# yurimjeon1892/EFGH

Measured on AMD Instinct MI355X. Metric: frame-pairs/sec EFGHNet fwd+bwd (384x1280 RGB + 64x2048 range), whole job, higher is better.
Workload: dtype f32; 1 GPU; BASELINE.json configs[2]: EFGHNet fwd+bwd with efghloss + gradient all-reduce + fused Adam, synthetic 384x1280 RGB + 131072-point sweep, batch=8 per GPU, random-init weights; global_batch=8, points=131072, parallelism=dp1

## Files before the change

### efgh_amd/csrc/gemm.hip

```cpp
#include "common.h"
#include <type_traits>

namespace {

typedef float f32x16 __attribute__((ext_vector_type(16)));
constexpr int BK = 32;
constexpr int LDS_LD = BK + 4;
struct KArgs {
    const float *A; int64_t lda;
    int C, T, K;
    unsigned magicC;
    int Hin, Win, Hv, Wv, sh, sw;
    unsigned long long dhpack, dwpack;
    int Ho, Wo, osh, osw, oh0, ow0;
    const int *table;
    const float *W; int N;
    int tld;
    long long M; const int *M_dev;
    const float *bias, *scale, *shift, *residual; int64_t ldr;
    int act; float slope;
    float *out; int64_t ldo;
    float *stats;
    unsigned nbx;
    unsigned nbatch;
// ... 73 lines not shown
    if (p.stats) {
#pragma unroll
        for (int j = 0; j < NI; ++j) {
            const int coll = (wn * NI + j) * 32 + l31;
            s1[j] += __shfl_xor(s1[j], 32); s2[j] += __shfl_xor(s2[j], 32);
            if (lh == 0) { ssum[wm * BN + coll] = s1[j]; ssq[wm * BN + coll] = s2[j]; }
        }
    }
    if (p.stats) {
        __syncthreads();
        for (int c = tid; c < BN; c += 256) {
            if (n0 + c < p.N) {
                float a = 0.f, b = 0.f;
#pragma unroll
                for (int w = 0; w < WM; ++w) { a += ssum[w * BN + c]; b += ssq[w * BN + c]; }
                p.stats[((long long)tile_m * 2 + 0) * p.N + n0 + c] = a;
                p.stats[((long long)tile_m * 2 + 1) * p.N + n0 + c] = b;
            }
        }
    }
}

template <int MODE, int BM, int BN, int WM, int WN>
__global__ void __launch_bounds__(256, 3)
k_gather_gemm(const KArgs p_in) {
    constexpr int MI = BM / WM / 32, NI = BN / WN / 32;
    constexpr int NA = BM / 32, NB = BN / 32;
    __shared__ __attribute__((aligned(16))) float As[BM * LDS_LD];
    __shared__ __attribute__((aligned(16))) float Bs[BN * LDS_LD];
    __shared__ long long rowout[BM];

    KArgs p = p_in;
    if (blockIdx.y) {
        p.A += blockIdx.y * p.bsA; p.W += blockIdx.y * p.bsW; p.out += blockIdx.y * p.bsO;
        if (MODE == 2) p.table += blockIdx.y * p.bsT;
    }
    const int tid = threadIdx.x, lane = tid & 63, wave = tid >> 6;
    const int wm = wave / WN, wn = wave % WN;
    const int l31 = lane & 31, lh = lane >> 5;
    long long M = p.M;
    if (p.M_dev) { long long md = *p.M_dev; M = md < M ? md : M; }
    const unsigned nbx = p.nbx, nblk = gridDim.x;
    const unsigned q8 = nblk >> 3, r8 = nblk & 7, xcd = blockIdx.x & 7, within = blockIdx.x >> 3;
    const unsigned lin = (xcd < r8 ? xcd * (q8 + 1) : r8 * (q8 + 1) + (xcd - r8) * q8) + within;
    const unsigned tile_m = lin / nbx, tile_n = lin - tile_m * nbx;
    const long long m0 = (long long)tile_m * BM;
    const int n0 = tile_n * BN;
    if (m0 >= M) return;

    const int arow = tid >> 3, kv = (tid & 7) * 4;
    long long abase[NA];
    unsigned amask[NA];
#pragma unroll
    for (int q = 0; q < NA; ++q) {
        long long m = m0 + q * 32 + arow;
        const bool ok = m < M;
        abase[q] = 0;
        amask[q] = 0;
        if (ok) {
            if (MODE == 0) { abase[q] = m * p.lda; amask[q] = 1; }
            else if (MODE == 4) { abase[q] = m * p.tld; amask[q] = 1; }
            else if (MODE == 2) {
                abase[q] = m * 16;
                amask[q] = 0xFFFFu;
                if (p.tam) amask[q] = (0x7FFFu & ~(unsigned)p_in.table[m * 16 + 15]) >> (blockIdx.y * p.bsT);
            }
// ... 108 lines not shown
            for (int i = 0; i < MI; ++i)
                a[i] = *reinterpret_cast<const float4 *>(
                    &As[((wm * MI + i) * 32 + l31) * LDS_LD + g * 8 + lh * 4]);
#pragma unroll
            for (int j = 0; j < NI; ++j)
                b[j] = *reinterpret_cast<const float4 *>(
                    &Bs[((wn * NI + j) * 32 + l31) * LDS_LD + g * 8 + lh * 4]);
#pragma unroll
            for (int i = 0; i < MI; ++i)
#pragma unroll
                for (int j = 0; j < NI; ++j) {
                    acc[i][j] = __builtin_amdgcn_mfma_f32_32x32x2f32(a[i].x, b[j].x, acc[i][j], 0, 0, 0);
                    acc[i][j] = __builtin_amdgcn_mfma_f32_32x32x2f32(a[i].y, b[j].y, acc[i][j], 0, 0, 0);
                    acc[i][j] = __builtin_amdgcn_mfma_f32_32x32x2f32(a[i].z, b[j].z, acc[i][j], 0, 0, 0);
                    acc[i][j] = __builtin_amdgcn_mfma_f32_32x32x2f32(a[i].w, b[j].w, acc[i][j], 0, 0, 0);
                }
        }
        __syncthreads();
    }

    gemm_epilogue<MODE, BM, BN, WM, WN>(p, M, m0, n0, tile_m, acc, rowout, As, wm, wn, l31, lh, tid);
}

__device__ __attribute__((aligned(128))) float g_gemm_zero[32];

constexpr int DMA_BM = 128;

template <int MODE, int BN>
__global__ void __launch_bounds__(256, 2)
k_gather_gemm_dma(const KArgs p_in) {
    constexpr int BM = DMA_BM, WM = 2, WN = 2, MI = 2, NI = BN / WN / 32, NBP = BN / 32;
    constexpr int STAGE = (BM + BN) * BK;
    extern __shared__ __attribute__((aligned(1024))) float ring[];
    __shared__ long long rowout[BM];

    KArgs p = p_in;
    if (blockIdx.y) { p.A += blockIdx.y * p.bsA; p.W += blockIdx.y * p.bsW; p.out += blockIdx.y * p.bsO; }
    const int tid = threadIdx.x, lane = tid & 63, wave = __builtin_amdgcn_readfirstlane(tid >> 6);
    const int wm = wave / WN, wn = wave % WN, l31 = lane & 31, lh = lane >> 5;
    const unsigned ring_lds = lds_addr(ring);
    const long long M = p.M;
    const unsigned nbx = p.nbx, nblk = gridDim.x;
    const unsigned q8 = nblk >> 3, r8 = nblk & 7, xcd = blockIdx.x & 7, within = blockIdx.x >> 3;
    const unsigned lin = (xcd < r8 ? xcd * (q8 + 1) : r8 * (q8 + 1) + (xcd - r8) * q8) + within;
    const unsigned tile_m = lin / nbx, tile_n = lin - tile_m * nbx;
    const long long m0 = (long long)tile_m * BM;
    const int n0 = tile_n * BN;
    if (m0 >= M) return;

    long long abase[4]; unsigned amask[4];
    const float *srcW[NBP];
    const int sub = lane >> 3;
#pragma unroll
    for (int q = 0; q < 4; ++q) {
        const int r = (wave * 4 + q) * 8 + sub;
        const int kq = (lane & 7) ^ ((r >> 1) & 7);
        const long long m = m0 + r;
        abase[q] = kq * 4; amask[q] = 0;
        if (m < M) {
            if (MODE == 0) { abase[q] += m * p.lda; amask[q] = 1; }
            else {
                const int j = (int)(m % p.Wv); const long long rr = m / p.Wv;
                const int i = (int)(rr % p.Hv); const long long b = rr / p.Hv;
                const int ih0 = i * p.sh, iw0 = j * p.sw;
                abase[q] += ((b * p.Hin + ih0) * p.Win + iw0) * p.lda;
                unsigned mk = 0;
// ... 77 lines not shown
        frag(0, a[0], b[0]);
#pragma unroll
        for (int g = 0; g < 4; ++g) {
            if (g < 3) frag(g + 1, a[(g + 1) & 1], b[(g + 1) & 1]);
            __builtin_amdgcn_sched_barrier(0);
            const float4 (&ca)[MI] = a[g & 1];
            const float4 (&cb)[NI] = b[g & 1];
#pragma unroll
            for (int i = 0; i < MI; ++i)
#pragma unroll
                for (int j = 0; j < NI; ++j) {
                    acc[i][j] = __builtin_amdgcn_mfma_f32_32x32x2f32(ca[i].x, cb[j].x, acc[i][j], 0, 0, 0);
                    acc[i][j] = __builtin_amdgcn_mfma_f32_32x32x2f32(ca[i].y, cb[j].y, acc[i][j], 0, 0, 0);
                    acc[i][j] = __builtin_amdgcn_mfma_f32_32x32x2f32(ca[i].z, cb[j].z, acc[i][j], 0, 0, 0);
                    acc[i][j] = __builtin_amdgcn_mfma_f32_32x32x2f32(ca[i].w, cb[j].w, acc[i][j], 0, 0, 0);
                }
            __builtin_amdgcn_sched_barrier(0);
        }
    }
    __syncthreads();
    gemm_epilogue<MODE, BM, BN, WM, WN>(p, M, m0, n0, tile_m, acc, rowout, ring, wm, wn, l31, lh, tid);
}

__global__ void k_pack_weight(const float *__restrict__ W, float *__restrict__ Wp, int N, int T, int C, int Nw, int Cw,
                              long long sn, long long sc, long long st, const int4 taps0,
                              const int4 taps1, const int4 taps2, const int4 taps3) {
    const int tp[16] = {taps0.x, taps0.y, taps0.z, taps0.w, taps1.x, taps1.y, taps1.z, taps1.w,
                        taps2.x, taps2.y, taps2.z, taps2.w, taps3.x, taps3.y, taps3.z, taps3.w};
    long long total = (long long)N * T * C;
    for (long long i = (long long)blockIdx.x * blockDim.x + threadIdx.x; i < total;
         i += (long long)gridDim.x * blockDim.x) {
        int c = (int)(i % C); long long r = i / C;
        int t = (int)(r % T); int n = (int)(r / T);
        int ti = 0;
#pragma unroll
        for (int q = 0; q < 16; ++q) if (q == t) ti = tp[q];
        Wp[i] = (n < Nw && c < Cw) ? W[n * sn + c * sc + ti * st] : 0.f;
    }
}

__global__ void __launch_bounds__(256) k_pack_weight_batched(const efgh_pack_job *__restrict__ jobs, const long long *__restrict__ prefix,
                                                             int njobs, long long total) {
    __shared__ int job_s;
    for (long long i0 = (long long)blockIdx.x * 256; i0 < total; i0 += (long long)gridDim.x * 256) {
        if (threadIdx.x == 0) {
            int lo = 0, hi = njobs - 1;
// ... 102 lines not shown
    const long long nby = (a.M + DMA_BM - 1) / DMA_BM;
    const size_t lds = (size_t)2 * (DMA_BM + BN) * BK * sizeof(float);
    if (!efgh_raise_lds_once(g_dma_raised[MODE * 2 + (BN == 128)], (const void *)k_gather_gemm_dma<MODE, BN>, (int)lds)) {
        efgh_set_error("%s:%d: cannot raise the dynamic LDS limit of k_gather_gemm_dma", __FILE__, __LINE__);
        return EFGH_E_LAUNCH;
    }
    k_gather_gemm_dma<MODE, BN><<<dim3((unsigned)(a.nbx * nby), a.nbatch), 256, lds, st>>>(a);
    return EFGH_OK;
}

template <int MODE>
int dispatch(const KArgs &a, hipStream_t st) {
    if constexpr (MODE == 0 || MODE == 1) {
        if (dma_ok(a, MODE)) return a.N > 64 ? launch_dma<MODE, 128>(a, st) : launch_dma<MODE, 64>(a, st);
    }
    if (a.N > 64) launch<MODE, 128, 128, 2, 2>(a, st);
    else if (a.N > 32) launch<MODE, 128, 64, 2, 2>(a, st);
    else launch<MODE, 256, 32, 4, 1>(a, st);
    return EFGH_OK;
}

int tile_m(int N) { return N > 32 ? 128 : 256; }

}

extern "C" int32_t efgh_gather_gemm_grid_m(int64_t M, int32_t N) {
    int bm = tile_m(N);
    return (int32_t)((M + bm - 1) / bm);
}

static int fill_args(const efgh_gemm_desc *d, KArgs &a, int tld = 0) {
    EFGH_CHECK_ARG(d && d->A && d->W && d->out);
    EFGH_CHECK_ARG(d->C > 0 && d->C % 4 == 0 && d->T >= 1 && (d->T <= 16 || d->mode == 3 || tld > 0));
    EFGH_CHECK_ARG(d->N >= 1 && d->M >= 1 && d->lda % 4 == 0);
    EFGH_CHECK_ARG((((uintptr_t)d->A) & 15) == 0 && (((uintptr_t)d->W) & 15) == 0);
    EFGH_CHECK_ARG(d->mode >= 0 && d->mode <= 3);
    EFGH_CHECK_ARG((int64_t)d->T * d->C < 65536);
    a.A = d->A; a.lda = d->lda; a.C = d->C; a.T = d->T; a.K = d->T * d->C;
    a.magicC = (unsigned)((0x100000000ULL + d->C - 1) / d->C);
    a.Hin = d->Hin; a.Win = d->Win; a.Hv = d->Hv; a.Wv = d->Wv; a.sh = d->sh; a.sw = d->sw;
    a.dhpack = 0; a.dwpack = 0;
    for (int t = 0; t < 16; ++t) {
        int dh = t < d->T ? d->dh[t] : 0, dw = t < d->T ? d->dw[t] : 0;
        if (d->mode == 1) EFGH_CHECK_ARG(dh >= -8 && dh <= 7 && dw >= -8 && dw <= 7);
        a.dhpack |= (unsigned long long)((dh + 8) & 15) << (4 * t);
        a.dwpack |= (unsigned long long)((dw + 8) & 15) << (4 * t);
// ... 13 lines not shown
    }
    a.tld = tld;
    if (tld > 0) EFGH_CHECK_ARG(d->mode == 2 && d->table != nullptr && tld >= d->T && a.nbatch == 1 && !d->table_alias_mask);
    else if (d->mode == 2) EFGH_CHECK_ARG(d->table != nullptr && d->batch_stride_table >= 0 && (int64_t)d->batch_stride_table * (a.nbatch - 1) + d->T <= 16);
    if (d->mode == 0) EFGH_CHECK_ARG(d->T == 1);
    if (d->mode == 3) EFGH_CHECK_ARG(d->B > 0 && d->Hin == d->T && d->Win > 0 && d->Wv > 0 && d->M == (int64_t)d->B * d->Wv);
    return EFGH_OK;
}

extern "C" int efgh_gather_gemm(const efgh_gemm_desc *d, void *stream_) {
    hipStream_t st = (hipStream_t)stream_;
    KArgs a;
    int rc = fill_args(d, a);
    if (rc != EFGH_OK) return rc;
    if (d->mode == 0) rc = dispatch<0>(a, st);
    else if (d->mode == 1) rc = dispatch<1>(a, st);
    else if (d->mode == 2) rc = dispatch<2>(a, st);
    else rc = dispatch<3>(a, st);
    if (rc != EFGH_OK) return rc;
    EFGH_CHECK_LAUNCH();
    return EFGH_OK;
}

extern "C" int efgh_blur_r_gemm(const efgh_gemm_desc *d, int32_t ld, void *stream_) {
    KArgs a;
    EFGH_CHECK_ARG(d && ld > 0);
    int rc = fill_args(d, a, ld);
    if (rc != EFGH_OK) return rc;
    rc = dispatch<4>(a, (hipStream_t)stream_);
    if (rc != EFGH_OK) return rc;
    EFGH_CHECK_LAUNCH();
    return EFGH_OK;
}

extern "C" int efgh_gather_gemm_set_dma(int32_t on) {
    const int old = g_use_dma ? 1 : 0;
    g_use_dma = on != 0;
    return old;
}

extern "C" int efgh_pack_weight_batched(const efgh_pack_job *jobs_dev, const int64_t *prefix_dev, int32_t njobs, int64_t total,
                                        void *stream_) {
    EFGH_CHECK_ARG(jobs_dev && prefix_dev && njobs > 0 && total > 0);
    long long g = (total + 255) / 256;
    k_pack_weight_batched<<<(int)(g > 16384 ? 16384 : g), 256, 0, (hipStream_t)stream_>>>(jobs_dev, (const long long *)prefix_dev, njobs,
                                                                                         total);
// ... 53 lines not shown
```

### efgh_amd/nets/fn.py

```python
import torch

from .. import ops
from ..ops import ACT_NONE, ceil4


def rows_ok(t):
    if t.stride(-1) != 1:
        return False
    ld = t.stride(-2) if t.dim() >= 2 else t.shape[-1]
    exp = ld
    for d in range(t.dim() - 2, -1, -1):
        if t.shape[d] != 1 and t.stride(d) != exp:
            return False
        exp *= t.shape[d]
    return ld % 4 == 0 and t.data_ptr() % 16 == 0


def as_rows(t):
    return t if rows_ok(t) else t.contiguous()


def ld_of(t):
    return t.stride(-2) if t.dim() >= 2 else t.shape[-1]


class LayerSpec:
    dgrad = custom_forward = custom_wgrad = None
    takes_bnsrc = passthrough = pool = defer_act = bwd_fusable = False

    def __init__(self, N, C, T, mode, launches, layouts, M, out_shape, bn=None, train=False, act=ACT_NONE, slope=0.0, table=None,
                 c_real=None):
        self.N, self.C, self.T, self.mode, self.M = N, C, T, mode, M
        self.launches, self.layouts, self.out_shape = launches, layouts, out_shape
        self.bn, self.train, self.act, self.slope, self.table = bn, train, act, slope, table
        self.c_real = c_real if c_real is not None else C

    def for_tape(self, dgrad, takes_bnsrc=False, custom_forward=None, custom_wgrad=None, passthrough=False, pool=False,
                 defer_act=False, bwd_fusable=False):
        self.dgrad, self.takes_bnsrc = dgrad, takes_bnsrc
        self.custom_forward, self.custom_wgrad = custom_forward, custom_wgrad
        self.passthrough = passthrough
        self.pool = pool
        self.defer_act = defer_act
        self.bwd_fusable = bwd_fusable
        return self


def run_launches(spec, x, lda, weight, out, ldo, bias, want_stats, a_off=0, out_off=0, lazy=None, pool=False, keep_on=None, **epilogue):
    Np = ceil4(spec.N)
    wps = [lay.pack(weight) for lay in spec.layouts]
    custom = spec.custom_forward
    stats, thin = None, False
    if want_stats:
        thin = custom is not None or ops.no_stats_epilogue(spec.mode, spec.C, Np, spec.T, spec.launches)
        if not thin:
            gs = [ops.stats_rows(spec.mode, spec.C, Np, g, m) for g, m in spec.launches]
            stats = torch.empty((sum(gs), 2, Np), dtype=torch.float32, device=x.device)
    if custom is not None:
        custom(x, weight, out)
    g0 = 0
    for li, (geom, m) in enumerate(spec.launches if custom is None else ()):
        T = ops.taps_of(spec.T, geom)
        st = None
        if stats is not None:
            st = stats[g0:g0 + gs[li]]
            g0 += gs[li]
        slot = None if keep_on is None else []
        ops.gather_gemm(x, lda, spec.C, T, wps[li], Np, m, out, ldo, mode=spec.mode, geom=geom, table=spec.table, bias=bias, stats=st,
                        a_off=a_off, out_off=out_off, flops=2.0 * m * spec.N * T * spec.c_real, lazy=lazy, pool=pool, keep_v=slot,
                        **epilogue)
        if slot and ops.wgrad_route(spec.mode, spec.C, Np, T, geom) == 'wino2d':
            if keep_on.kept_v is None:
                keep_on.kept_v = {}
            keep_on.kept_v[li] = slot[0]
    if thin:
        stats, _ = ops.col_stats(out, spec.M, Np, ldo, x_off=out_off)
    return stats


def bn_batch_stats(bn, stats, Np, count, save=False):
    N = bn.num_features
    ops.bn_tick(bn)
    momentum = bn.momentum if bn.momentum is not None else 0.1
    rm, rv = ops.pad_vec(bn.running_mean, Np), ops.pad_vec(bn.running_var, Np, 1.0)
# ... 608 lines not shown
```

### efgh_amd/nets/fnet.py

```python
import math
import os

import torch
import torch.nn as nn

from .. import ops
from ..common import pose
from . import fn as FN
from . import layers as L
from .builders import VGGFeatures, conv_bn_relu, convt_bn_relu


class Fnet(nn.Module):
    def __init__(self, args):
        super().__init__()
        self.device = args['DEVICE']
        raw = args['raw_cam_img_size']
        self.range_img_size = (int(raw[0] / 2), int(raw[1] * 2))
        self.lidar_fov_rad = args['lidar_fov_rad']
        self.vgg_camera = VGGFeatures('C')
        self.vgg_5_1_camera = convt_bn_relu(512, 128, (3, 3), (2, 2), 1)
        self.vgg_5_2_camera = convt_bn_relu(128, 32, (3, 3), (2, 2), 0)
        self.vgg_5_3_camera = convt_bn_relu(32, 16, (3, 3), (2, 2), 1)
        self.conv_range = conv_bn_relu(4, 3, (1, 2), (1, 1), 0)
        self.vgg_range = VGGFeatures('C')
        self.vgg_5_1_range = convt_bn_relu(512, 128, (3, 3), (2, 2), 1)
        self.vgg_5_2_range = convt_bn_relu(128, 32, (3, 3), (2, 2), 0)
        self.vgg_5_3_range = convt_bn_relu(32, 16, (3, 3), (2, 2), 1)

    def _trunk(self, ctx, x, side):
        x = L.run_vgg(ctx, getattr(self, 'vgg_' + side).features, x)
        x = L.run_convt_bn_relu(ctx, getattr(self, 'vgg_5_1_' + side), x)
        x = L.run_convt_bn_relu(ctx, getattr(self, 'vgg_5_2_' + side), x)
        return L.run_convt_bn_relu(ctx, getattr(self, 'vgg_5_3_' + side), x)

    def forward(self, pc, ret, check=False, keep=None, cam_stream=None):
        ctx = L.Ctx(self.training)
        H, W = self.range_img_size
        fov = (self.lidar_fov_rad[0] * math.pi, self.lidar_fov_rad[1] * math.pi)
        if ctx.grad:
            e_range = FN.RangeImageFn.apply(pc, ret['e_l'], H, W, fov[0], fov[1])
        else:
            e_range, _ = ops.range_image(pc, ret['e_l'], H, W, fov[0], fov[1])
        from . import efghbackbone as bb
        main = torch.cuda.current_stream() if pc.is_cuda else None

        def camera():
            h_img = ret.get('_h_img_nhwc')
            if h_img is None:
                h_img = ops.nchw_to_nhwc(ret['h_img'], 4)
            return self._trunk(ctx, h_img, 'camera')

        def rng_branch():
            r0 = L.run_conv_bn_relu(ctx, self.conv_range, e_range)
            return self._trunk(ctx, r0, 'range')
        if cam_stream is not None:
            rng = rng_branch()
            with torch.cuda.stream(cam_stream):
                cam = camera()
            main.wait_stream(cam_stream)
# ... 18 lines not shown
```

### efgh_amd/nets/gnet.py

```python
import torch
import torch.nn as nn

from .. import ops
from ..common import pose
from . import fn as FN
from . import layers as L
from .builders import conv_bn_relu, convt_bn_relu, resnet18_layers

import os as _os
HEADS_FUSED = True


class Gnet(nn.Module):
    def __init__(self, args):
        super().__init__()
        self.device = args['DEVICE']
        self.raw_cam_img_size = args['raw_cam_img_size']
        self.conv_i0 = conv_bn_relu(3, 64, 3, 1, 1)
        self.conv_img2, self.conv_img3, self.conv_img4, self.conv_img5 = resnet18_layers()
        self.convt_img4 = convt_bn_relu(512, 256, 3, 2, 1, 1)
        self.convt_img3 = convt_bn_relu(512, 128, 3, 2, 1, 1)
        self.convt_img2 = convt_bn_relu(256, 64, 3, 2, 1, 1)
        self.convt_dimg = convt_bn_relu(128, 1, 3, 2, 1, 1)
        self.convt_mask = convt_bn_relu(128, 2, 3, 2, 1, 1)
        self.conv_i1 = conv_bn_relu(64, 32, 1, 1, 0)
        self.conv_d1 = conv_bn_relu(4, 32, 3, 2, 1)
        self.conv2, self.conv3, self.conv4, self.conv5 = resnet18_layers()
        self.conv_trs_1 = conv_bn_relu(512, 512, 1)
        self.conv_trs_2 = conv_bn_relu(512, 512, 1)
        self.conv_trs_3 = conv_bn_relu(512, 512, 1)
        self.conv_trs_4 = nn.Conv1d(512, 3, 1)

    def image_part(self, img, img_nhwc=None):
        ctx = L.Ctx(self.training)
        dev = img.device
        x = img_nhwc if img_nhwc is not None else ops.nchw_to_nhwc(img, 4)
        B, H, W, _ = x.shape

        def buf(h, w, c):
            return torch.empty((B, h, w, c), dtype=torch.float32, device=dev)

        def tgt(b, off):
            return (b, off)

        def cat(b, parts):
            return FN.concat(b, parts) if ctx.grad else b
        assert H % 2 == 0 and W % 8 == 0, 'reference needs raw H % 4 == 0 and (W/2) % 8 == 0 (SURVEY 8a-17)'
        h2, h3 = (H + 1) // 2, ((H + 1) // 2 + 1) // 2

        def crop(t, h, b, off):
            if t.shape[1] == h:
                return t
            t = t[:, :h]
            if not ctx.grad:
                b[..., off:off + t.shape[-1]].copy_(t)
            return t
        cat0_box = []
# ... 26 lines not shown
        else:
            L.run_conv_bn_relu(ctx, self.conv_i1, cat1, out=(cat0_early(), 0), in_ch=(0, 64))
        ready = None
        if x.is_cuda:
            ready = torch.cuda.Event()
            ready.record()
        cv = cat(cat1, [t2, c2])
        cat0 = cat0_early()
        if HEADS_FUSED and x.is_cuda and L.convt_heads_fusable(self.convt_dimg, self.convt_mask):
            hm = L.run_convt_heads(ctx, self.convt_dimg, self.convt_mask, cv)
            g_depth, g_mask = FN.HeadsToNchwFn.apply(hm) if ctx.grad else ops.heads_to_nchw(hm)
        else:
            dimg, cv = L.run_convt_bn_relu(ctx, self.convt_dimg, cv, skip_out=True)
            mask = L.run_convt_bn_relu(ctx, self.convt_mask, cv)
            if ctx.grad:
                g_depth = FN.NhwcToNchwFn.apply(dimg, 1)
                g_mask = FN.Softmax2ToNchwFn.apply(mask)
            else:
                g_depth = ops.nhwc_to_nchw(dimg, 1)
                g_mask = ops.softmax2_to_nchw(mask)
        return {'g_depth': g_depth, 'g_mask': g_mask, 'ci1': ci1, 'cat0': cat0, 'ready': ready}

    def forward(self, pc, img, ret, check=False, img_nhwc=None, keep=None, pre=None):
        ctx = L.Ctx(self.training)
        if pre is None:
            pre = self.image_part(img, img_nhwc)
        g_depth, g_mask, ci1, cat0 = pre['g_depth'], pre['g_mask'], pre['ci1'], pre['cat0']
        B = cat0.shape[0]

        def tgt(b, off):
            return (b, off)
        rawH, rawW = self.raw_cam_img_size
        if ctx.grad:
            f_depth = FN.DepthImageFn.apply(pc, ret['efh_cam_T_velo'], rawH, rawW)
        else:
            f_depth, _ = ops.depth_image(pc, ret['efh_cam_T_velo'], rawH, rawW)
        if ctx.grad:
            cd1 = L.run_conv_bn_relu(ctx, self.conv_d1, f_depth, out=tgt(cat0, 32))
            y = FN.concat(cat0, [ci1, cd1])
        else:
            L.run_conv_bn_relu(ctx, self.conv_d1, f_depth, out=(cat0, 32))
            y = cat0
        y = L.run_resnet_layer(ctx, self.conv2, y)
        y = L.run_resnet_layer(ctx, self.conv3, y)
        y = L.run_resnet_layer(ctx, self.conv4, y)
        y = L.run_resnet_layer(ctx, self.conv5, y)
        for seq in (self.conv_trs_1, self.conv_trs_2, self.conv_trs_3):
# ... 25 lines not shown
```

### efgh_amd/nets/layers.py

```python
import itertools

import torch
import torch.nn as nn
import torch.nn.functional as F

from .. import lattice, ops
from ..ops import ACT_LEAKY, ACT_NONE, ACT_RELU, ceil4
from . import fn as FN


class Ctx:

    def __init__(self, train):
        self.train = bool(train)
        self.grad = torch.is_grad_enabled()


def _bn_eval_affine(bn, Np):
    key = ('bn_eval', Np)
    vers = ops._ver(bn.weight, bn.bias, bn.running_mean, bn.running_var) + \
        ((bn.num_batches_tracked._version,) if bn.num_batches_tracked is not None else ())

    def make():
        with torch.no_grad():
            scale = bn.weight.detach() * torch.rsqrt(bn.running_var + bn.eps)
            shift = bn.bias.detach() - bn.running_mean * scale
        return ops.pad_vec(scale, Np), ops.pad_vec(shift, Np)

    return ops._cached(bn, key, vers, make)


def _bias_vec(bias, Np):
    if bias is None:
        return None
    if bias.numel() == Np:
        return bias.detach()
    return ops._cached(bias, ('bias', Np), ops._ver(bias), lambda: ops.pad_vec(bias, Np))

# ... 62 lines not shown
           defer_act=False):
    B, H, W, ldx = x.shape
    Cw, O = conv.in_channels, conv.out_channels
    kh, kw = conv.kernel_size
    sh, sw = conv.stride
    ph, pw = conv.padding
    a_off, Cx = in_ch if in_ch is not None else (0, ldx)
    Cp = ceil4(Cw)
    assert Cx == Cp, (Cx, Cw)
    Ho, Wo = (H + 2 * ph - kh) // sh + 1, (W + 2 * pw - kw) // sw + 1
    T = kh * kw
    Np = ceil4(O)
    dh = [i // kw - ph for i in range(T)]
    dw = [i % kw - pw for i in range(T)]
    geom = (B, H, W, Ho, Wo, sh, sw, dh, dw, Ho, Wo, 1, 1, 0, 0)
    M = B * Ho * Wo
    lay = ops.WeightLayout(O, T, Cw, Cw * T, T, 1, list(range(T)), Np, Cp, ('conv', Np, Cp))
    spec = FN.LayerSpec(O, Cp, T, 1, [(geom, M)], [lay], M, (B, Ho, Wo), bn=bn, train=ctx.train, act=act, slope=slope, c_real=Cw)
    if ctx.grad:
        assert in_ch is None or getattr(x, '_efgh_lazy', None) is None
        xs = x if in_ch is None else x[..., a_off:a_off + Cx]
        fus = bool((kh, kw, sh, sw, ph, pw) == (3, 3, 1, 1, 1, 1) and bn is not None and ctx.train
                   and ops.lazy_capable(1, Np, Cp, _same3x3_geom(B, H, W)) and ops.wgrad_lazy_capable(1, Cp, Np, geom))
        spec.for_tape(_conv2d_dgrad(conv, (B, H, W, Ho, Wo), Np, Cp), takes_bnsrc=True,
                      passthrough=skip_out and xs.requires_grad and xs.shape[-1] == Cp, pool=pool, defer_act=defer_act, bwd_fusable=fus)
        return _apply(spec, xs, conv.weight, conv.bias, residual, skip_out, out)
    assert not defer_act
    if pool:
        assert out is None and residual is None and not ctx.train
        out_t, ldo, coff = _alloc_out(x, (B, Ho if pool == 'h' else Ho // 2, Wo // 2), O, None)
        _run(ctx, spec, x, ldx, conv.weight, conv.bias, out_t, ldo, coff, a_off=a_off, pool=pool)
        return ops.maxpool_v2(out_t) if pool == 'h' else out_t
    out_t, ldo, coff = _alloc_out(x, (B, Ho, Wo), O, out)
    res_ld = residual.shape[-1] if residual is not None else 0
    _run(ctx, spec, x, ldx, conv.weight, conv.bias, out_t, ldo, coff, residual=residual, res_ld=res_ld, a_off=a_off)
    return out_t


def _conv2d_dgrad(conv, dims, Np, Cp):
    B, H, W, Ho, Wo = dims
    Cw, O = conv.in_channels, conv.out_channels
    kh, kw = conv.kernel_size
    sh, sw = conv.stride
    ph, pw = conv.padding
    T = kh * kw

    def dgrad(spec, w, draw, xin, add=None, bnsrc=None, pre_v=None):
        dev = (draw if draw is not None else pre_v).device
        ldr = 0 if add is None else FN.ld_of(add)
        assert pre_v is None or (sh == 1 and sw == 1)
        if sh == 1 and sw == 1:
            order = sorted(range(T), key=lambda i: (ph - i // kw, pw - i % kw))
            dhs = [ph - i // kw for i in order]
            dws = [pw - i % kw for i in order]
            Wd = ops.WeightLayout(Cw, T, O, T, Cw * T, 1, order, Cp, Np, ('conv_d', Np, Cp)).pack(w)
            dx = torch.empty((B, H, W, Cp), dtype=torch.float32, device=dev)
            g = (B, Ho, Wo, H, W, 1, 1, dhs, dws, H, W, 1, 1, 0, 0)
            st = ops.gather_gemm(draw, Np, Np, T, Wd, Cp, B * H * W, dx, Cp, mode=1, geom=g, residual=add, ldr=ldr,
                                 flops=2.0 * B * H * W * Cw * T * O, bn_bwd=bnsrc, pre_v=pre_v)
            if st is not None:
                dx._efgh_bnsums = (st, bnsrc, dx._version)
            return dx
        assert sh == 2 and sw == 2
        classes = list(_parity_classes(kh, kw, ph, pw, H, W))
        if add is not None and len(classes) < 4:
            dx, ldx_ = add, ldr
            assert add.shape[-1] == Cp
        elif len(classes) == 4:
            dx, ldx_ = torch.empty((B, H, W, Cp), dtype=torch.float32, device=dev), Cp
        else:
            dx, ldx_ = torch.zeros((B, H, W, Cp), dtype=torch.float32, device=dev), Cp
        for cy, cx, tapidx, Hv, Wv, dhs, dws in classes:
            Wd = ops.WeightLayout(Cw, len(tapidx), O, T, Cw * T, 1, tapidx, Cp, Np, ('conv_d2', cy, cx, Np, Cp)).pack(w)
            g = (B, Ho, Wo, Hv, Wv, 1, 1, dhs, dws, H, W, 2, 2, cy, cx)
            ops.gather_gemm(draw, Np, Np, len(tapidx), Wd, Cp, B * Hv * Wv, dx, ldx_, mode=1, geom=g, residual=add, ldr=ldr,
                            flops=2.0 * B * Hv * Wv * Cw * len(tapidx) * O)
        return dx
    return dgrad


def _convt_wcol(convt):
    Cw, O = convt.in_channels, convt.out_channels
    w = convt.weight

    def make():
        wd = w.detach().reshape(Cw, O, 9).permute(2, 1, 0).reshape(9 * O, Cw)
        full = torch.zeros((ceil4(9 * O), Cw), dtype=torch.float32, device=wd.device)
        full[:9 * O] = wd
        return full
    return ops._cached(w, ('wcol',), ops._ver(w), make)


def _convt_small_forward(x, convt, out_raw, scale=None, shift=None, act=ACT_NONE, slope=0.0):
    B, H, W, Cw = x.shape
    O = convt.out_channels
    Ho, Wo = out_raw.shape[1], out_raw.shape[2]
    wcol = _convt_wcol(convt)
    Y = torch.empty((B * H * W, wcol.shape[0]), dtype=torch.float32, device=x.device)
    ops.gather_gemm(x, FN.ld_of(x), Cw, 1, wcol, wcol.shape[0], B * H * W, Y, wcol.shape[0], mode=0,
# ... 6 lines not shown
    Cw, O = convt.in_channels, convt.out_channels
    assert convt.kernel_size == (3, 3) and convt.stride == (2, 2) and ldx == Cw and Cw % 4 == 0
    ph, pw = convt.padding
    oph, opw = convt.output_padding
    Ho, Wo = (H - 1) * 2 - 2 * ph + 3 + oph, (W - 1) * 2 - 2 * pw + 3 + opw
    Np = ceil4(O)
    small = O <= 3 and ph == pw and convt.bias is None and bn is not None
    if small and out is None and not ctx.grad:
        out_t = torch.empty((B, Ho, Wo, 4), dtype=torch.float32, device=x.device)
        if not ctx.train:
            sc, sh = _bn_eval_affine(bn, 4)
            _convt_small_forward(x, convt, out_t, sc, sh, act, slope)
        else:
            _convt_small_forward(x, convt, out_t)
            stats, _ = ops.col_stats(out_t, B * Ho * Wo, 4, 4)
            scale, shift, _, _ = FN.bn_batch_stats(bn, stats, 4, float(B * Ho * Wo))
            ops.scale_shift_act(out_t, 4, scale, shift, out_t, 4, B * Ho * Wo, 4, act, slope)
        return out_t
    launches, layouts = [], []
    for cy, cx, tapidx, Hv, Wv, dh, dw in _parity_classes(3, 3, ph, pw, Ho, Wo):
        launches.append(((B, H, W, Hv, Wv, 1, 1, dh, dw, Ho, Wo, 2, 2, cy, cx), B * Hv * Wv))
        layouts.append(ops.WeightLayout(O, len(tapidx), Cw, 9, O * 9, 1, tapidx, Np, key=('convt', cy, cx, ph, pw, Np)))
    spec = FN.LayerSpec(O, Cw, 0, 1, launches, layouts, B * Ho * Wo, (B, Ho, Wo), bn=bn, train=ctx.train, act=act, slope=slope)
    if ctx.grad:
        assert out is None
        cfwd, cwgrad = _convt_small_grad(convt, (B, H, W, Ho, Wo)) if small else (None, None)
        spec.for_tape(_convt_dgrad(convt, (B, H, W, Ho, Wo)), custom_forward=cfwd, custom_wgrad=cwgrad,
                      passthrough=skip_out and x.requires_grad,
                      defer_act=not small and defer_for is not None and lazy_consumer_ok(ctx, defer_for, B, Ho, Wo))
        return _apply(spec, x, convt.weight, convt.bias, None, skip_out)
    out_t, ldo, coff = _alloc_out(x, (B, Ho, Wo), O, out)
    _run(ctx, spec, x, ldx, convt.weight, convt.bias, out_t, ldo, coff)
    return out_t


def _convt_dgrad(convt, dims):
    B, H, W, Ho, Wo = dims
    Cw, O = convt.in_channels, convt.out_channels
    ph, pw = convt.padding
    Np = ceil4(O)

    def dgrad(spec, w, draw, xin, add=None):
        dhs = [k // 3 - ph for k in range(9)]
        dws = [k % 3 - pw for k in range(9)]
        Wd = ops.WeightLayout(Cw, 9, O, O * 9, 9, 1, list(range(9)), Cp=Np, key=('convt_d', Np)).pack(w)
        dx = torch.empty((B, H, W, Cw), dtype=torch.float32, device=draw.device)
# ... 367 lines not shown
```

### efgh_amd/ops.py

```python
import ctypes
import os as _os
import threading
import weakref

import torch

from . import _C
from ._C import c_float, ptr

ACT_NONE, ACT_RELU, ACT_LEAKY = 0, 1, 2


def _L():
    return _C.lib()


def _st():
    return _C.stream_ptr()


def ceil4(n):
    return (n + 3) // 4 * 4


# ... 576 lines not shown
    elif route == 'sc':
        _C.check(_L().efgh_sc_conv3x3(ctypes.byref(d), _st()))
    elif route == 'wino2d':
        if (bn_bwd is not None and stats is None and BN_BWD_FUSED_2D and out_off == 0 and not pool and bn_bwd.fits(M, N)
                and bn_bwd.y is None and bn_bwd.raw.stride(-2) % 4 == 0):
            rows = _L().efgh_wino2d_stats_rows(geom[0], geom[1], geom[2], N)
            bn_stats = _bn_bwd_sums(d, bn_bwd, rows, N, out.device)
        _wino2d_forward(d, A, a_off, lda, C, N, geom, Wp, pool=pool, lazy=lazy, pre_v=pre_v, keep_v=keep_v)
    elif route == 'wino_hpool':
        _C.check(_L().efgh_wino_conv3x3_hpool(ctypes.byref(d), ptr(wino_weight(Wp, N, C)), _st()))
    elif route == 'wino':
        if bn_bwd is not None and stats is None and BN_BWD_FUSED and out_off == 0 and bn_bwd.fits(M, N):
            rows = _L().efgh_wino_grid_m(geom[0], geom[1], geom[2])
            bn_stats = _bn_bwd_sums(d, bn_bwd, rows, N, out.device)
        _C.check(_L().efgh_wino_conv3x3(ctypes.byref(d), ptr(wino_weight(Wp, N, C)), _st()))
    else:
        _C.check(_L().efgh_gather_gemm(ctypes.byref(d), _st()))
    if ev is not None:
        _prof_end(ev, route, (mode, M, N, T, C), float(flops) if flops is not None else 2.0 * M * N * T * C, PROFILE, PROFILE_WINO,
                  batched=batch is not None)
    return bn_stats


def _bn_bwd_sums(d, src, rows, N, device):
    part = torch.empty((rows, 2, N), dtype=torch.float32, device=device)
    d.stats, d.stats_mode = part.data_ptr(), 1
    d.bn_raw, d.bn_ldraw = src.raw.data_ptr(), src.raw.stride(-2)
    if src.y is not None:
        d.bn_y, d.bn_ldy = src.y.data_ptr(), src.y.stride(-2)
    else:
        d.bn_pscale, d.bn_pshift = src.psc.data_ptr(), src.psh.data_ptr()
    d.bn_mean, d.bn_invstd = src.mean.data_ptr(), src.invstd.data_ptr()
    d.bn_act, d.bn_slope = src.act, src.slope
    return part


GEMM_DMA = True


def apply_switches():
    _L().efgh_gather_gemm_set_dma(1 if GEMM_DMA else 0)


PLANE_DMA = True
PLANE_DMA_NBUF = 0
PROFILE_WINO2D = None
# ... 1050 lines not shown
```

### include/efgh_hip.h

```cpp
#ifndef EFGH_HIP_H
#define EFGH_HIP_H
#include <stdint.h>

#ifdef __cplusplus
extern "C" {
#endif

#define EFGH_OK 0
#define EFGH_E_INVALID (-1)
#define EFGH_E_LAUNCH (-2)
#define EFGH_WROTE_OUT 1

const char *efgh_last_error(void);

#define EFGH_ABI_VERSION 4
int efgh_version(void);

#define EFGH_LATTICE_INFO_H 0
#define EFGH_LATTICE_INFO_ERR 1
#define EFGH_LATTICE_INFO_ALIAS 2
#define EFGH_LATTICE_INFO_CURSOR 3
#define EFGH_LATTICE_INFO_SEG 4
#define EFGH_LATTICE_MAX_SAMPLES 1024

// ... 57 lines not shown
    const int32_t *table;
    const float *W;
    int32_t N;
    int64_t M;
    const int32_t *M_dev;
    const float *bias, *scale, *shift;
    const float *residual; int64_t ldr;
    int32_t act;
    float slope;
    float *out; int64_t ldo;
    float *stats;
    int32_t nbatch;
    int64_t batch_stride_a, batch_stride_w, batch_stride_out;
    int32_t batch_stride_table;
    int32_t table_alias_mask;
    int32_t stats_mode;
    const float *bn_raw; int64_t bn_ldraw;
    const float *bn_y; int64_t bn_ldy;
    const float *bn_pscale, *bn_pshift, *bn_mean, *bn_invstd;
    int32_t bn_act; float bn_slope;
} efgh_gemm_desc;

int efgh_gather_gemm(const efgh_gemm_desc *d, void *stream);
int efgh_bwd_finalize_f32(const float *stats, int32_t rows, int32_t C, double count, float *sum_dpre, float *sum_dpre_xhat,
                          double *mean_dpre, double *mean_dpre_xhat, void *stream);
int32_t efgh_gather_gemm_grid_m(int64_t M, int32_t N);

int efgh_pack_weight(const float *W, float *Wp, int32_t N, int32_t T, int32_t C, int64_t sn,
                     int64_t sc, int64_t st, const int32_t *tapidx_host, void *stream);
int efgh_pack_weight_padded(const float *W, float *Wp, int32_t N, int32_t T, int32_t C, int32_t Np, int32_t Cp, int64_t sn,
                            int64_t sc, int64_t st, const int32_t *tapidx_host, void *stream);
typedef struct {
    const float *W; float *Wp;
    int32_t N, T, C, Np, Cp, pad_;
    int64_t sn, sc, st;
    int32_t taps[16];
} efgh_pack_job;
int efgh_pack_weight_batched(const efgh_pack_job *jobs_dev, const int64_t *prefix_dev, int32_t njobs, int64_t total, void *stream);
int efgh_pack_weight_batched_tiled(const efgh_pack_job *jobs_dev, const int64_t *tile_prefix_dev, int32_t njobs, int64_t ntiles,
                                   void *stream);
int efgh_fold_planes(const float *part, int32_t S, int64_t M, int32_t N, const float *bias, int32_t act, float slope, float *out,
                     int64_t ldo, void *stream);
int efgh_pad_vec(const float *v, int32_t n, float *out, int32_t np, float fill, void *stream);


int efgh_bn_finalize(const float *stats, int32_t G, int32_t C, double count, const float *gamma,
// ... 409 lines not shown
```

Before: 31.40 frame-pairs/s.

## Merge stride-2 parity-class GEMM launches into one multi-class kernel launch

Stride-2 conv dgrad and transposed-conv forward currently issue one gather-GEMM launch per parity class (up to four). A class-table kernel now maps each block to its class, sorted by K so the heavier classes go first, and runs all classes in a single launch with per-class weights, geometry and stats. The aim is to cut launch overhead and tail idle time between small launches. In exchange it adds a larger kernel-argument struct and per-block class lookup, and the whole grid must share one tile configuration.

```diff
diff --git a/efgh_amd/csrc/gemm.hip b/efgh_amd/csrc/gemm.hip
--- a/efgh_amd/csrc/gemm.hip
+++ b/efgh_amd/csrc/gemm.hip
@@ -1,4 +1,5 @@
 #include "common.h"
+#include <algorithm>
 #include <type_traits>
 
 namespace {
@@ -119,8 +120,7 @@
 }
 
 template <int MODE, int BM, int BN, int WM, int WN>
-__global__ void __launch_bounds__(256, 3)
-k_gather_gemm(const KArgs p_in) {
+__device__ __forceinline__ void gather_gemm_body(const KArgs &p_in, const unsigned bid, const unsigned nblk) {
     constexpr int MI = BM / WM / 32, NI = BN / WN / 32;
     constexpr int NA = BM / 32, NB = BN / 32;
     __shared__ __attribute__((aligned(16))) float As[BM * LDS_LD];
@@ -137,8 +137,8 @@
     const int l31 = lane & 31, lh = lane >> 5;
     long long M = p.M;
     if (p.M_dev) { long long md = *p.M_dev; M = md < M ? md : M; }
-    const unsigned nbx = p.nbx, nblk = gridDim.x;
-    const unsigned q8 = nblk >> 3, r8 = nblk & 7, xcd = blockIdx.x & 7, within = blockIdx.x >> 3;
+    const unsigned nbx = p.nbx;
+    const unsigned q8 = nblk >> 3, r8 = nblk & 7, xcd = bid & 7, within = bid >> 3;
     const unsigned lin = (xcd < r8 ? xcd * (q8 + 1) : r8 * (q8 + 1) + (xcd - r8) * q8) + within;
     const unsigned tile_m = lin / nbx, tile_n = lin - tile_m * nbx;
     const long long m0 = (long long)tile_m * BM;
@@ -293,13 +293,18 @@
     gemm_epilogue<MODE, BM, BN, WM, WN>(p, M, m0, n0, tile_m, acc, rowout, As, wm, wn, l31, lh, tid);
 }
 
+template <int MODE, int BM, int BN, int WM, int WN>
+__global__ void __launch_bounds__(256, 3)
+k_gather_gemm(const KArgs p_in) {
+    gather_gemm_body<MODE, BM, BN, WM, WN>(p_in, blockIdx.x, gridDim.x);
+}
+
 __device__ __attribute__((aligned(128))) float g_gemm_zero[32];
 
 constexpr int DMA_BM = 128;
 
 template <int MODE, int BN>
-__global__ void __launch_bounds__(256, 2)
-k_gather_gemm_dma(const KArgs p_in) {
+__device__ __forceinline__ void gather_gemm_dma_body(const KArgs &p_in, const unsigned bid, const unsigned nblk) {
     constexpr int BM = DMA_BM, WM = 2, WN = 2, MI = 2, NI = BN / WN / 32, NBP = BN / 32;
     constexpr int STAGE = (BM + BN) * BK;
     extern __shared__ __attribute__((aligned(1024))) float ring[];
@@ -311,8 +316,8 @@
     const int wm = wave / WN, wn = wave % WN, l31 = lane & 31, lh = lane >> 5;
     const unsigned ring_lds = lds_addr(ring);
     const long long M = p.M;
-    const unsigned nbx = p.nbx, nblk = gridDim.x;
-    const unsigned q8 = nblk >> 3, r8 = nblk & 7, xcd = blockIdx.x & 7, within = blockIdx.x >> 3;
+    const unsigned nbx = p.nbx;
+    const unsigned q8 = nblk >> 3, r8 = nblk & 7, xcd = bid & 7, within = bid >> 3;
     const unsigned lin = (xcd < r8 ? xcd * (q8 + 1) : r8 * (q8 + 1) + (xcd - r8) * q8) + within;
     const unsigned tile_m = lin / nbx, tile_n = lin - tile_m * nbx;
     const long long m0 = (long long)tile_m * BM;
@@ -436,6 +441,57 @@
     gemm_epilogue<MODE, BM, BN, WM, WN>(p, M, m0, n0, tile_m, acc, rowout, ring, wm, wn, l31, lh, tid);
 }
 
+template <int MODE, int BN>
+__global__ void __launch_bounds__(256, 2)
+k_gather_gemm_dma(const KArgs p_in) {
+    gather_gemm_dma_body<MODE, BN>(p_in, blockIdx.x, gridDim.x);
+}
+
+constexpr int MAX_CLASSES = 4;
+struct KClass {
+    const float *W; float *stats;
+    unsigned long long dhpack, dwpack;
+    long long M;
+    int T, K, Hv, Wv, osh, osw, oh0, ow0;
+};
+struct KClasses {
+    KClass c[MAX_CLASSES];
+    unsigned first[MAX_CLASSES];
+    unsigned count[MAX_CLASSES];
+    int n;
+};
+
+__device__ __forceinline__ void take_class(KArgs &p, const KClasses &cl, unsigned &bid, unsigned &nblk) {
+    const unsigned b = blockIdx.x;
+    int ci = 0;
+#pragma unroll
+    for (int i = 1; i < MAX_CLASSES; ++i) ci += (i < cl.n && b >= cl.first[i]) ? 1 : 0;
+    ci = __builtin_amdgcn_readfirstlane(ci);
+    const KClass &k = cl.c[ci];
+    p.W = k.W; p.stats = k.stats; p.dhpack = k.dhpack; p.dwpack = k.dwpack; p.M = k.M;
+    p.T = k.T; p.K = k.K; p.Hv = k.Hv; p.Wv = k.Wv; p.osh = k.osh; p.osw = k.osw; p.oh0 = k.oh0; p.ow0 = k.ow0;
+    bid = b - cl.first[ci];
+    nblk = cl.count[ci];
+}
+
+template <int BM, int BN, int WM, int WN>
+__global__ void __launch_bounds__(256, 3)
+k_gather_gemm_classes(const KArgs p_in, const KClasses cl) {
+    KArgs p = p_in;
+    unsigned bid, nblk;
+    take_class(p, cl, bid, nblk);
+    gather_gemm_body<1, BM, BN, WM, WN>(p, bid, nblk);
+}
+
+template <int BN>
+__global__ void __launch_bounds__(256, 2)
+k_gather_gemm_dma_classes(const KArgs p_in, const KClasses cl) {
+    KArgs p = p_in;
+    unsigned bid, nblk;
+    take_class(p, cl, bid, nblk);
+    gather_gemm_dma_body<1, BN>(p, bid, nblk);
+}
+
 __global__ void k_pack_weight(const float *__restrict__ W, float *__restrict__ Wp, int N, int T, int C, int Nw, int Cw,
                               long long sn, long long sc, long long st, const int4 taps0,
                               const int4 taps1, const int4 taps2, const int4 taps3) {
@@ -584,6 +640,40 @@
 
 int tile_m(int N) { return N > 32 ? 128 : 256; }
 
+template <int BM, int BN, int WM, int WN>
+void launch_classes(const KArgs &a0, KClasses &cl, hipStream_t st) {
+    KArgs a = a0;
+    a.nbx = (unsigned)((a.N + BN - 1) / BN);
+    unsigned total = 0;
+    for (int i = 0; i < cl.n; ++i) {
+        cl.first[i] = total;
+        cl.count[i] = (unsigned)(a.nbx * ((cl.c[i].M + BM - 1) / BM));
+        total += cl.count[i];
+    }
+    k_gather_gemm_classes<BM, BN, WM, WN><<<dim3(total, 1), 256, 0, st>>>(a, cl);
+}
+
+std::atomic<unsigned long long> g_dma_classes_raised[2];
+
+template <int BN>
+int launch_dma_classes(const KArgs &a0, KClasses &cl, hipStream_t st) {
+    KArgs a = a0;
+    a.nbx = (unsigned)((a.N + BN - 1) / BN);
+    unsigned total = 0;
+    for (int i = 0; i < cl.n; ++i) {
+        cl.first[i] = total;
+        cl.count[i] = (unsigned)(a.nbx * ((cl.c[i].M + DMA_BM - 1) / DMA_BM));
+        total += cl.count[i];
+    }
+    const size_t lds = (size_t)2 * (DMA_BM + BN) * BK * sizeof(float);
+    if (!efgh_raise_lds_once(g_dma_classes_raised[BN == 128], (const void *)k_gather_gemm_dma_classes<BN>, (int)lds)) {
+        efgh_set_error("%s:%d: cannot raise the dynamic LDS limit of k_gather_gemm_dma_classes", __FILE__, __LINE__);
+        return EFGH_E_LAUNCH;
+    }
+    k_gather_gemm_dma_classes<BN><<<dim3(total, 1), 256, lds, st>>>(a, cl);
+    return EFGH_OK;
+}
+
 }
 
 extern "C" int32_t efgh_gather_gemm_grid_m(int64_t M, int32_t N) {
@@ -643,6 +733,51 @@
     return EFGH_OK;
 }
 
+extern "C" int efgh_gather_gemm_classes(const efgh_gemm_desc *c0, const efgh_gemm_desc *c1, const efgh_gemm_desc *c2,
+                                        const efgh_gemm_desc *c3, int32_t nclasses, void *stream_) {
+    hipStream_t st = (hipStream_t)stream_;
+    const efgh_gemm_desc *classes[MAX_CLASSES] = {c0, c1, c2, c3};
+    EFGH_CHECK_ARG(nclasses >= 1 && nclasses <= MAX_CLASSES);
+    for (int i = 0; i < nclasses; ++i) EFGH_CHECK_ARG(classes[i] != nullptr);
+    KArgs a[MAX_CLASSES];
+    for (int i = 0; i < nclasses; ++i) {
+        const efgh_gemm_desc *d = classes[i], *s = classes[0];
+        EFGH_CHECK_ARG(d->mode == 1 && !d->M_dev && d->nbatch <= 1 && d->stats_mode == 0);
+        int rc = fill_args(d, a[i]);
+        if (rc != EFGH_OK) return rc;
+        EFGH_CHECK_ARG(d->A == s->A && d->lda == s->lda && d->C == s->C && d->N == s->N && d->out == s->out && d->ldo == s->ldo);
+        EFGH_CHECK_ARG(d->B == s->B && d->Hin == s->Hin && d->Win == s->Win && d->Ho == s->Ho && d->Wo == s->Wo && d->sh == s->sh
+                       && d->sw == s->sw);
+        EFGH_CHECK_ARG(d->bias == s->bias && d->scale == s->scale && d->shift == s->shift && d->residual == s->residual
+                       && d->ldr == s->ldr && d->act == s->act && d->slope == s->slope && !d->stats == !s->stats);
+    }
+    int order[MAX_CLASSES];
+    for (int i = 0; i < nclasses; ++i) order[i] = i;
+    std::stable_sort(order, order + nclasses, [&](int x, int y) { return a[x].K > a[y].K; });
+    long long wgs = 0;
+    for (int i = 0; i < nclasses; ++i) wgs += ((a[i].M + 127) / 128) * ((a[i].N + 31) / 32);
+    EFGH_CHECK_ARG(wgs < 0x7fffffffLL);
+    KClasses cl = {};
+    cl.n = nclasses;
+    bool dma = true;
+    for (int i = 0; i < nclasses; ++i) {
+        const KArgs &k = a[order[i]];
+        KClass &c = cl.c[i];
+        c.W = k.W; c.stats = k.stats; c.dhpack = k.dhpack; c.dwpack = k.dwpack; c.M = k.M;
+        c.T = k.T; c.K = k.K; c.Hv = k.Hv; c.Wv = k.Wv; c.osh = k.osh; c.osw = k.osw; c.oh0 = k.oh0; c.ow0 = k.ow0;
+        dma = dma && dma_ok(k, 1);
+    }
+    const KArgs &s = a[0];
+    int rc = EFGH_OK;
+    if (dma) rc = s.N > 64 ? launch_dma_classes<128>(s, cl, st) : launch_dma_classes<64>(s, cl, st);
+    else if (s.N > 64) launch_classes<128, 128, 2, 2>(s, cl, st);
+    else if (s.N > 32) launch_classes<128, 64, 2, 2>(s, cl, st);
+    else launch_classes<256, 32, 4, 1>(s, cl, st);
+    if (rc != EFGH_OK) return rc;
+    EFGH_CHECK_LAUNCH();
+    return EFGH_OK;
+}
+
 extern "C" int efgh_blur_r_gemm(const efgh_gemm_desc *d, int32_t ld, void *stream_) {
     KArgs a;
     EFGH_CHECK_ARG(d && ld > 0);
diff --git a/efgh_amd/nets/fn.py b/efgh_amd/nets/fn.py
--- a/efgh_amd/nets/fn.py
+++ b/efgh_amd/nets/fn.py
@@ -27,6 +27,7 @@
 class LayerSpec:
     dgrad = custom_forward = custom_wgrad = None
     takes_bnsrc = passthrough = pool = defer_act = bwd_fusable = False
+    one_launch = False
 
     def __init__(self, N, C, T, mode, launches, layouts, M, out_shape, bn=None, train=False, act=ACT_NONE, slope=0.0, table=None,
                  c_real=None):
@@ -59,7 +60,16 @@
     if custom is not None:
         custom(x, weight, out)
     g0 = 0
-    for li, (geom, m) in enumerate(spec.launches if custom is None else ()):
+    one = (spec.one_launch and custom is None and lazy is None and not pool
+           and ops.classes_one_launch(spec.mode, spec.C, Np, spec.launches, stats is not None))
+    if one:
+        sts = None
+        if stats is not None:
+            ends = [sum(gs[:li + 1]) for li in range(len(gs))]
+            sts = [stats[e - g:e] for e, g in zip(ends, gs)]
+        ops.gather_gemm_classes(x, lda, spec.C, wps, Np, spec.launches, out, ldo, bias=bias, stats=sts, a_off=a_off, out_off=out_off,
+                                flops=sum(2.0 * m * spec.N * ops.taps_of(spec.T, g) * spec.c_real for g, m in spec.launches), **epilogue)
+    for li, (geom, m) in enumerate(spec.launches if custom is None and not one else ()):
         T = ops.taps_of(spec.T, geom)
         st = None
         if stats is not None:
diff --git a/efgh_amd/nets/fnet.py b/efgh_amd/nets/fnet.py
--- a/efgh_amd/nets/fnet.py
+++ b/efgh_amd/nets/fnet.py
@@ -35,7 +35,7 @@
         return L.run_convt_bn_relu(ctx, getattr(self, 'vgg_5_3_' + side), x)
 
     def forward(self, pc, ret, check=False, keep=None, cam_stream=None):
-        ctx = L.Ctx(self.training)
+        ctx = L.Ctx(self.training, one_launch=True)
         H, W = self.range_img_size
         fov = (self.lidar_fov_rad[0] * math.pi, self.lidar_fov_rad[1] * math.pi)
         if ctx.grad:
diff --git a/efgh_amd/nets/gnet.py b/efgh_amd/nets/gnet.py
--- a/efgh_amd/nets/gnet.py
+++ b/efgh_amd/nets/gnet.py
@@ -32,7 +32,7 @@
         self.conv_trs_4 = nn.Conv1d(512, 3, 1)
 
     def image_part(self, img, img_nhwc=None):
-        ctx = L.Ctx(self.training)
+        ctx = L.Ctx(self.training, one_launch=True)
         dev = img.device
         x = img_nhwc if img_nhwc is not None else ops.nchw_to_nhwc(img, 4)
         B, H, W, _ = x.shape
@@ -105,7 +105,7 @@
         return {'g_depth': g_depth, 'g_mask': g_mask, 'ci1': ci1, 'cat0': cat0, 'ready': ready}
 
     def forward(self, pc, img, ret, check=False, img_nhwc=None, keep=None, pre=None):
-        ctx = L.Ctx(self.training)
+        ctx = L.Ctx(self.training, one_launch=True)
         if pre is None:
             pre = self.image_part(img, img_nhwc)
         g_depth, g_mask, ci1, cat0 = pre['g_depth'], pre['g_mask'], pre['ci1'], pre['cat0']
diff --git a/efgh_amd/nets/layers.py b/efgh_amd/nets/layers.py
--- a/efgh_amd/nets/layers.py
+++ b/efgh_amd/nets/layers.py
@@ -11,9 +11,10 @@
 
 class Ctx:
 
-    def __init__(self, train):
+    def __init__(self, train, one_launch=False):
         self.train = bool(train)
         self.grad = torch.is_grad_enabled()
+        self.one_launch = bool(one_launch)
 
 
 def _bn_eval_affine(bn, Np):
@@ -122,7 +123,7 @@
         xs = x if in_ch is None else x[..., a_off:a_off + Cx]
         fus = bool((kh, kw, sh, sw, ph, pw) == (3, 3, 1, 1, 1, 1) and bn is not None and ctx.train
                    and ops.lazy_capable(1, Np, Cp, _same3x3_geom(B, H, W)) and ops.wgrad_lazy_capable(1, Cp, Np, geom))
-        spec.for_tape(_conv2d_dgrad(conv, (B, H, W, Ho, Wo), Np, Cp), takes_bnsrc=True,
+        spec.for_tape(_conv2d_dgrad(conv, (B, H, W, Ho, Wo), Np, Cp, ctx.one_launch), takes_bnsrc=True,
                       passthrough=skip_out and xs.requires_grad and xs.shape[-1] == Cp, pool=pool, defer_act=defer_act, bwd_fusable=fus)
         return _apply(spec, xs, conv.weight, conv.bias, residual, skip_out, out)
     assert not defer_act
@@ -137,7 +138,7 @@
     return out_t
 
 
-def _conv2d_dgrad(conv, dims, Np, Cp):
+def _conv2d_dgrad(conv, dims, Np, Cp, one_launch=False):
     B, H, W, Ho, Wo = dims
     Cw, O = conv.in_channels, conv.out_channels
     kh, kw = conv.kernel_size
@@ -170,11 +171,16 @@
             dx, ldx_ = torch.empty((B, H, W, Cp), dtype=torch.float32, device=dev), Cp
         else:
             dx, ldx_ = torch.zeros((B, H, W, Cp), dtype=torch.float32, device=dev), Cp
-        for cy, cx, tapidx, Hv, Wv, dhs, dws in classes:
-            Wd = ops.WeightLayout(Cw, len(tapidx), O, T, Cw * T, 1, tapidx, Cp, Np, ('conv_d2', cy, cx, Np, Cp)).pack(w)
-            g = (B, Ho, Wo, Hv, Wv, 1, 1, dhs, dws, H, W, 2, 2, cy, cx)
-            ops.gather_gemm(draw, Np, Np, len(tapidx), Wd, Cp, B * Hv * Wv, dx, ldx_, mode=1, geom=g, residual=add, ldr=ldr,
-                            flops=2.0 * B * Hv * Wv * Cw * len(tapidx) * O)
+        lays = [ops.WeightLayout(Cw, len(tapidx), O, T, Cw * T, 1, tapidx, Cp, Np, ('conv_d2', cy, cx, Np, Cp))
+                for cy, cx, tapidx, Hv, Wv, dhs, dws in classes]
+        launches = [((B, Ho, Wo, Hv, Wv, 1, 1, dhs, dws, H, W, 2, 2, cy, cx), B * Hv * Wv) for cy, cx, tapidx, Hv, Wv, dhs, dws in classes]
+        flops = [2.0 * m * Cw * len(g[7]) * O for g, m in launches]
+        if one_launch and ops.classes_one_launch(1, Np, Cp, launches):
+            ops.gather_gemm_classes(draw, Np, Np, [lay.pack(w) for lay in lays], Cp, launches, dx, ldx_, residual=add, ldr=ldr,
+                                    flops=sum(flops))
+            return dx
+        for lay, (g, m), fl in zip(lays, launches, flops):
+            ops.gather_gemm(draw, Np, Np, len(g[7]), lay.pack(w), Cp, m, dx, ldx_, mode=1, geom=g, residual=add, ldr=ldr, flops=fl)
         return dx
     return dgrad
 
@@ -227,6 +233,7 @@
         launches.append(((B, H, W, Hv, Wv, 1, 1, dh, dw, Ho, Wo, 2, 2, cy, cx), B * Hv * Wv))
         layouts.append(ops.WeightLayout(O, len(tapidx), Cw, 9, O * 9, 1, tapidx, Np, key=('convt', cy, cx, ph, pw, Np)))
     spec = FN.LayerSpec(O, Cw, 0, 1, launches, layouts, B * Ho * Wo, (B, Ho, Wo), bn=bn, train=ctx.train, act=act, slope=slope)
+    spec.one_launch = ctx.one_launch
     if ctx.grad:
         assert out is None
         cfwd, cwgrad = _convt_small_grad(convt, (B, H, W, Ho, Wo)) if small else (None, None)
diff --git a/efgh_amd/ops.py b/efgh_amd/ops.py
--- a/efgh_amd/ops.py
+++ b/efgh_amd/ops.py
@@ -622,6 +622,29 @@
     return bn_stats
 
 
+STRIDE2_ONE_LAUNCH = True
+
+
+def classes_one_launch(mode, C, N, launches, stats=False):
+    return bool(STRIDE2_ONE_LAUNCH and mode == 1 and 2 <= len(launches) <= 4
+                and all(g is not None and gemm_route(mode, C, N, len(g[7]), g, m, stats=stats) == 'gemm' for g, m in launches))
+
+
+def gather_gemm_classes(A, lda, C, Wps, N, launches, out, ldo, bias=None, scale=None, shift=None, residual=None, ldr=0, act=ACT_NONE,
+                        slope=0.0, stats=None, a_off=0, out_off=0, res_off=0, flops=None):
+    n = len(launches)
+    descs = [_desc(A, lda, C, len(geom[7]), 1, N, m, geom, None, a_off, Wps[i], out, ldo, out_off, bias, scale, shift, residual, ldr,
+                   res_off, act, slope, None if stats is None else stats[i]) for i, (geom, m) in enumerate(launches)]
+    c = [ctypes.byref(d) for d in descs] + [None] * (4 - n)
+    ev = _prof_start(PROFILE)
+    _C.check(_L().efgh_gather_gemm_classes(c[0], c[1], c[2], c[3], n, _st()))
+    if ev is not None:
+        rows = sum(m for _, m in launches)
+        taps = round(sum(float(m) * len(g[7]) for g, m in launches) / rows, 2)
+        fl = float(flops) if flops is not None else sum(2.0 * m * N * len(g[7]) * C for g, m in launches)
+        _prof_end(ev, 'gemm', (1, rows, N, taps, C), fl, PROFILE, PROFILE_WINO)
+
+
 def _bn_bwd_sums(d, src, rows, N, device):
     part = torch.empty((rows, 2, N), dtype=torch.float32, device=device)
     d.stats, d.stats_mode = part.data_ptr(), 1
diff --git a/include/efgh_hip.h b/include/efgh_hip.h
--- a/include/efgh_hip.h
+++ b/include/efgh_hip.h
@@ -103,6 +103,8 @@
 } efgh_gemm_desc;
 
 int efgh_gather_gemm(const efgh_gemm_desc *d, void *stream);
+int efgh_gather_gemm_classes(const efgh_gemm_desc *c0, const efgh_gemm_desc *c1, const efgh_gemm_desc *c2, const efgh_gemm_desc *c3,
+                             int32_t nclasses, void *stream);
 int efgh_bwd_finalize_f32(const float *stats, int32_t rows, int32_t C, double count, float *sum_dpre, float *sum_dpre_xhat,
                           double *mean_dpre, double *mean_dpre_xhat, void *stream);
 int32_t efgh_gather_gemm_grid_m(int64_t M, int32_t N);
```

After: 31.42 frame-pairs/s (median of 2 runs). No clear change (+0.1%).
